# balazs-bamer/cuda-bezier-triangle-raytracer

Hardware: AMD Instinct MI355X
Metric: Mrays/sec (primary+refracted) at 1/2/4/8 MI355X; % of HBM-read roofline (higher is better)
Workload: dtype f32; 1 GPU; cfg4: two stacked cfg2 lenses at x=10 and x=13, 4096x4096 rays; image=4096x4096, primaries_per_gpu=16777216, patches=6144, parallelism=64x64 image tiles round-robin over 1 rank(s), strong scaling, pipeline=fused, frames_in_flight=3, scan=BVH-culled (bit-identical to brute force), numerics=parity: bit-identical to the CPU oracle

## Files before the change

cuda-bezier-triangle-raytracer_amd/bzr_amd/__init__.py:

```python
from __future__ import annotations

import ctypes
import os
from contextlib import contextmanager
from pathlib import Path

import numpy as np

PKG_DIR = Path(__file__).resolve().parent.parent
LIB_PATH = Path(os.environ.get("BZR_LIBRARY", PKG_DIR / "lib" / "libbzr.so"))

OK = 0
HOST_PTRS, DEVICE_PTRS = 0, 1
MODE_PARITY, MODE_FAST = 0, 2
ACCEL_NONE = 4
PIPELINE_STAGED = 8
PIPELINE_FUSED = 16
RAYS_AOS = 32
WHAT_FOLLOW0, WHAT_FOLLOW1, WHAT_FOLLOW2, WHAT_NONE, WHAT_INTERSECT = 0, 1, 2, 3, 4
LIMIT_THIS, LIMIT_NONE = 0, 1
RR_NONE, RR_INSIDE, RR_OUTSIDE = 0, 1, 2
ENVELOPE_ELLIPSOID, ENVELOPE_TESTLENS = 0, 1
PATCH_WORDS = 66
KERNELS = ("k_traverse", "bucket", "k_newton", "k_follow", "k_finish", "k_overflow", "k_intersect_scan",
           "k_refract_scan", "k_chain_scan", "k_patch", "k_newton_lane", "k_trace")
COUNTERS = ("segments", "pairs", "follows", "overflow_rays", "lane_chunks", "node_visits", "leaf_fetches",
            "gate_tests", "newton_rounds", "rounds_odd", "runs_odd", "short_passes")
HIT_FIELDS = 13

_P = ctypes.c_void_p
_U32 = ctypes.c_uint32
_I32 = ctypes.c_int32
_F = ctypes.c_float

_SIGS = {
    "bzr_abi_version": [],
    "bzr_last_error": [],
    "bzr_device_count": [ctypes.POINTER(_I32)],
    "bzr_ctx_create": [_I32, ctypes.POINTER(_P)],
    "bzr_ctx_destroy": [_P],
    "bzr_ctx_set_stream": [_P, _P],
    "bzr_ctx_use_own_stream": [_P],
    "bzr_ctx_get_stream": [_P, ctypes.POINTER(_P)],
    "bzr_sync": [_P],
    "bzr_ctx_timing": [_P, _I32],
    "bzr_ctx_timing_report": [_P, _P, _P],
    "bzr_ctx_counters": [_P, _I32],
    "bzr_ctx_counters_report": [_P, _P],
    "bzr_mesh_create": [_P, _P, _U32, _U32, ctypes.POINTER(_P)],
    "bzr_mesh_destroy": [_P],
    "bzr_mesh_size": [_P, ctypes.POINTER(_U32)],
    "bzr_intersect": [_P, _P, _P, _U32, _P, _U32],
    "bzr_intersect_records": [_P, _P, _P, _U32, _P, _P, _U32],
    "bzr_patch_intersect": [_P, _P, _P, _P, _P, _U32, _P, _U32],
    "bzr_refract": [_P, _P, _F, _P, _P, _U32, _U32, _P, _P, _U32],
    "bzr_trace_chain": [_P, _P, _P, _U32, _P, _U32, _P, _P, _P, _U32],
    "bzr_trace_chain_power": [_P, _P, _P, _U32, _P, _P, _U32, _P, _P, _P, _P, _U32],
    "bzr_trace_chain_spectral": [_P, _P, _P, _U32, _U32, _P, _P, _P, _U32, _P, _P, _P, _P, _U32],
    "bzr_trace_chain_tir": [_P, _P, _P, _U32, _U32, _P, _P, _P, _U32, _U32, _P, _P, _P, _P, _P, _U32],
    "bzr_trace_chain_opl": [_P, _P, _P, _U32, _U32, _P, _P, _P, _P, _U32, _U32, _P, _P, _P, _P, _P, _P, _P, _U32],
    "bzr_trace_chain_media": [_P, _P, _P, _P, _U32, _U32, _P, _P, _P, _P, _U32, _U32, _P, _P, _P, _P, _P, _P, _P, _U32],
    "bzr_dispersion_index": [_I32, _P, _U32, _P, _U32, _P],
    "bzr_trace_tiled": [_P, _U32, _P, _P, _U32, _P, _U32, _U32, _P, _P, _P, _U32],
    "bzr_tiled_create": [_P, _U32, _U32, _U32, _U32, _I32, ctypes.POINTER(_P)],
    "bzr_tiled_destroy": [_P],
    "bzr_tiled_info": [_P, _P, _P, _P],
    "bzr_tiled_set_rays": [_P, _P, _U32],
    "bzr_tiled_share_rays": [_P, _U32, ctypes.POINTER(_P)],
    "bzr_tiled_trace": [_P, _P, _P, _U32, _P, _P, _P, _U32],
    "bzr_tiled_stream": [_P, ctypes.POINTER(_P)],
    "bzr_tiled_sync": [_P],
    "bzr_tiled_set_layout": [_P, _I32, _U32],
    "bzr_tiled_calibrate": [_P, _P, _P, _U32, _U32, ctypes.POINTER(_U32)],
    "bzr_mesh_interpolate": [_P, _P, _I32, _P, _U32],
    "bzr_emit": [_P, _P, ctypes.c_uint64, _U32, _P, _P, _U32],
    "bzr_illuminate": [_P, _P, _P, _U32, _P, ctypes.c_uint64, _P, _P, _P, _U32],
    "bzr_illuminate_power": [_P, _P, _P, _U32, _P, ctypes.c_uint64, _P, _P, _P, _P, _P, _P, _U32],
    "bzr_illuminate_spectral": [_P, _P, _P, _U32, _U32, _P, ctypes.c_uint64, _P, _P, _P, _P, _P, _P, _U32],
    "bzr_illuminate_tir": [_P, _P, _P, _U32, _U32, _P, ctypes.c_uint64, _P, _P, _U32, _P, _P, _P, _P, _P, _P, _P, _P,
                           _U32],
    "bzr_mesh_bounding_sphere": [_P, _P],
    "bzr_trimesh_create": [ctypes.POINTER(_P)],
    "bzr_trimesh_destroy": [_P],
    "bzr_trimesh_copy": [_P, ctypes.POINTER(_P)],
    "bzr_trimesh_size": [_P, ctypes.POINTER(_U32)],
    "bzr_trimesh_get": [_P, _P],
    "bzr_trimesh_set": [_P, _P, _U32],
    "bzr_trimesh_make_solid_of_revolution": [_P, _I32, _I32, _I32, _F, _F, _F],
    "bzr_trimesh_make_ellipsoid": [_P, _I32, _I32, _F, _F, _F],
    "bzr_trimesh_read_stl": [_P, ctypes.c_char_p],
    "bzr_trimesh_write_stl": [_P, ctypes.c_char_p],
    "bzr_trimesh_transform": [_P, _P, _P],
    "bzr_trimesh_split": [_P, _I32],
    "bzr_trimesh_split_maxside": [_P, _F],
    "bzr_trimesh_standardize_vertices": [_P],
    "bzr_trimesh_standardize_normals": [_P],
    "bzr_trimesh_neighbours": [_P, _P, _P],
    "bzr_bezier_build": [_P, _P],
    "bzr_bezier_split_thick": [_P, _P],
    "bzr_bezier_interpolate": [_P, _I32, _P],
    "bzr_pack_frame": [_P, _I32, _P, _P, _P, _U32, _U32, _U32, _P],
    "bzr_debug_unit": [_P, _P, _U32, _P],
    "bzr_debug_div_heights": [_P, _P, _U32, _P],
    "bzr_debug_bundle_setup": [_P, _P, _P, _U32, _P],
    "bzr_debug_fast_unit": [_P, _P, _U32, _P],
    "bzr_debug_wave_clock": [_P, _P, _U32],
    "bzr_debug_wave_clock_rate": [_P, _P, _U32],
    "bzr_debug_chunk_plan": [ctypes.c_uint64, ctypes.c_uint64, ctypes.POINTER(_U32), ctypes.POINTER(_U32)],
    "bzr_debug_chunk_cap": [_P, _U32, ctypes.POINTER(_U32)],
    "bzr_debug_fresnel": [_P, _P, _U32, _P],
}
_ADDED = ("bzr_trace_chain_power", "bzr_illuminate_power", "bzr_trace_chain_spectral", "bzr_illuminate_spectral",
          "bzr_dispersion_index", "bzr_trace_chain_tir", "bzr_illuminate_tir", "bzr_trace_chain_opl",
          "bzr_trace_chain_media")
_RET = {"bzr_last_error": ctypes.c_char_p, "bzr_abi_version": _I32}

_lib = None


class BzrError(RuntimeError):
    pass


def lib():
    global _lib
    if _lib is None:
        if os.environ.get("BZR_NO_TORCH_PRELOAD") != "1":
            try:
                import torch
            except ImportError:
                pass
        if not LIB_PATH.exists():
            raise BzrError(f"{LIB_PATH} is missing: build it with `python -c 'import __graft_entry__ as g; g.build()'`")
        handle = ctypes.CDLL(str(LIB_PATH))
        for name, args in _SIGS.items():
            if (os.environ.get("BZR_LIBRARY") and (name.startswith("bzr_debug_") or name in _ADDED)
                    and not hasattr(handle, name)):
                continue
            fn = getattr(handle, name)
            fn.argtypes = args
            fn.restype = _RET.get(name, _I32)
        _lib = handle
    return _lib


def exported_symbols():
    return list(_SIGS)


def _check(status: int):
    if status != OK:
        msg = lib().bzr_last_error().decode(errors="replace")
        raise BzrError(f"libbzr status {status}: {msg}")


def device_count() -> int:
    c = _I32(0)
    _check(lib().bzr_device_count(ctypes.byref(c)))
    return c.value


def _is_tensor(x) -> bool:
    return hasattr(x, "data_ptr") and hasattr(x, "is_cuda")


class _Buf:

    def __init__(self, x, dtype, writable=False):
        if x is None:
            self.ptr, self.device, self.keep = None, None, None
            return
        if _is_tensor(x):
            if not x.is_contiguous():
                raise BzrError("tensor arguments must be contiguous")
            want = {np.float32: "torch.float32", np.uint32: "torch.uint32", np.int32: "torch.int32",
                    np.uint64: "torch.uint64", np.uint8: "torch.uint8"}
            same_bits = {np.uint32: "torch.int32", np.uint64: "torch.int64"}
            if str(x.dtype) not in (want[dtype], same_bits.get(dtype, want[dtype])):
                raise BzrError(f"tensor dtype {x.dtype} where {want[dtype]} is expected")
            self.ptr, self.device, self.keep = x.data_ptr(), bool(x.is_cuda), x
        else:
            a = np.asarray(x)
            if a.dtype != dtype or not a.flags["C_CONTIGUOUS"]:
                if writable:
                    raise BzrError(f"output array must be C-contiguous {np.dtype(dtype).name}")
                a = np.ascontiguousarray(a, dtype=dtype)
            self.ptr, self.device, self.keep = a.ctypes.data, False, a
# ... 756 lines not shown
```

cuda-bezier-triangle-raytracer_amd/csrc/device/patch_math.hpp:

```cpp
#pragma once
#include <hip/hip_runtime.h>
#include <cfloat>
#include <cstdint>

namespace bzr_dev {

struct f3 {
  float x, y, z;
};
__device__ __forceinline__ f3 mk(float x, float y, float z) { return f3{x, y, z}; }
namespace rec {
constexpr int kUnder = 0;
constexpr int kDivider = 4;
constexpr int kNeigh = 16;
constexpr int kCp = 19;
constexpr int kMinv = 49;
constexpr int kHin = 58;
constexpr int kHout = 59;
constexpr int kDirA = 60;
constexpr int kDirB = 63;
constexpr int kWords = 66;
}

struct Patch {
// ... 73 lines not shown
#ifndef BZR_NEWTON_UNROLL
#define BZR_NEWTON_UNROLL 1
#endif
constexpr uint32_t kFollow2 = 2u, kNone = 3u, kIntersect = 4u;

namespace exact {
__device__ __forceinline__ float div_rn(float a, float b) { return a / b; }
__device__ __forceinline__ float sqrt_rn(float a) { return __builtin_sqrtf(a); }

__device__ __forceinline__ float sqrt_unscaled(float z) {
  const float s = __builtin_amdgcn_sqrtf(z);
  const float lo = __uint_as_float(__float_as_uint(s) - 1u), hi = __uint_as_float(__float_as_uint(s) + 1u);
  const float rlo = __builtin_fmaf(-lo, s, z), rhi = __builtin_fmaf(-hi, s, z);
  const float t = rlo <= 0.0f ? lo : s;
  return rhi > 0.0f ? hi : t;
}
__device__ __forceinline__ float div_unscaled(float a, float b, float y) {
  float q = a * y;
  float r = __builtin_fmaf(-b, q, a);
  q = __builtin_fmaf(r, y, q);
  r = __builtin_fmaf(-b, q, a);
  return __builtin_fmaf(r, y, q);
}
__device__ __forceinline__ bool sqrt_above_hundredth(float z) { return z > __uint_as_float(0x38d1b718u); }
__device__ __forceinline__ f3 unit_or_self(f3 a, float z) {
  const float s = sqrt_unscaled(z);
  const float y0 = __builtin_amdgcn_rcpf(s);
  const float y = __builtin_fmaf(__builtin_fmaf(-s, y0, 1.0f), y0, y0);
  f3 r = mk(div_unscaled(a.x, s, y), div_unscaled(a.y, s, y), div_unscaled(a.z, s, y));
  const float m = fminf(fminf(fabsf(a.x), fabsf(a.y)), fabsf(a.z));
  if (!(m >= 0x1p-100f && z >= 0x1p-96f && z <= 0x1p40f)) {
    r = a;
    if (z > 0.0f) {
      const float sr = sqrt_rn(z);
      r = mk(div_rn(a.x, sr), div_rn(a.y, sr), div_rn(a.z, sr));
    }
  }
  return r;
}
#ifndef BZR_DIV_HEIGHTS
#define BZR_DIV_HEIGHTS 1
#endif
__device__ __forceinline__ bool height_in_range(float h) {
  const uint32_t e = (__float_as_uint(h) >> 23) & 0xFFu;
  return e - (127u - 40u) <= 80u;
}
__device__ __forceinline__ void div_heights(float hin, float hout, float ic, float &din, float &dout) {
#if BZR_DIV_HEIGHTS
  const bool ok = height_in_range(hin) && height_in_range(hout) && fabsf(ic) >= 0x1p-20f && fabsf(ic) <= 0x1p20f;
  if (__all(ok)) {
    const float y0 = __builtin_amdgcn_rcpf(ic);
    const float y = __builtin_fmaf(__builtin_fmaf(-ic, y0, 1.0f), y0, y0);
    din = div_unscaled(hin, ic, y);
    dout = div_unscaled(hout, ic, y);
    return;
  }
#endif
  din = div_rn(hin, ic);
  dout = div_rn(hout, ic);
}
#include "patch_math_body.inc"
}

namespace fast {
#pragma clang fp contract(fast)
__device__ __forceinline__ float div_rn(float a, float b) { return a * __builtin_amdgcn_rcpf(b); }
__device__ __forceinline__ float sqrt_rn(float a) { return __builtin_amdgcn_sqrtf(a); }
__device__ __forceinline__ bool sqrt_above_hundredth(float z) { return sqrt_rn(z) > 0.01f; }
__device__ __forceinline__ f3 unit_or_self(f3 a, float z) {
  if (!(z > 0.0f)) return a;
  float r = __builtin_amdgcn_rsqf(z);
  return mk(a.x * r, a.y * r, a.z * r);
}
__device__ __forceinline__ void div_heights(float hin, float hout, float ic, float &din, float &dout) {
  din = div_rn(hin, ic);
  dout = div_rn(hout, ic);
}
#include "patch_math_body.inc"
#pragma clang fp contract(off)
}

using namespace exact;

template <bool kGated = false, bool kFast = false, typename P, typename Need = NormalAlways>
__device__ __forceinline__ Hit patch_intersect(const P &p, f3 s, f3 d, bool limitNone, Need need = Need()) {
  Hit h;
  h.t = 0.0f;
  h.point = mk(0.0f, 0.0f, 0.0f);
  h.cs = 0.0f;
  h.bary = h.point;
  h.normal = h.point;
  h.what = kNone;
  f3 ip;
  float ic, it;
  bool valid = plane_ray(p.n(), p.c(), s, d, ip, ic, it);
  (void)valid;
  if (!kGated) {
    if (!(valid && fabsf(it) > -p.hin() && fabsf(it) > p.hout())) return h;
    f3 b0 = matvec(p, ip);
    if (!(limitNone || (b0.x >= 0.0f && b0.x <= 1.0f && b0.y >= 0.0f && b0.y <= 1.0f && b0.z >= 0.0f && b0.z <= 1.0f)))
      return h;
  }
  if constexpr (kFast) return fast::newton_tail(p, s, d, ic, it, need);
  else return newton_tail(p, s, d, ic, it, need);
}

}
```

cuda-bezier-triangle-raytracer_amd/csrc/device/trace.hip:

```cpp
#include <hip/hip_runtime.h>
#include <hipcub/hipcub.hpp>

#include <algorithm>
#include <climits>
#include <cmath>
#include <cstdlib>

#include <cstdio>
#include <cstring>
#include <new>
#include <type_traits>
#include <string>
#include <vector>

#include "../host/bvh.hpp"
#include "../host/staging.hpp"
#include "bzr.h"
#include "ctx.hpp"
#include "patch_math.hpp"
#include "emitter.hpp"

using namespace bzr_dev;

namespace {
thread_local std::string t_error;
bzr_status set_error(bzr_status s, const std::string &msg) {
  t_error = msg;
  return s;
}
#define BZR_HIP(call)                                                                                     \
  do {                                                                                                    \
    hipError_t e_ = (call);                                                                               \
    if (e_ != hipSuccess) return set_error(BZR_ERR_HIP, std::string(#call ": ") + hipGetErrorString(e_)); \
  } while (0)
}

extern "C" const char *bzr_last_error(void) { return t_error.c_str(); }
extern "C" int32_t bzr_abi_version(void) { return BZR_ABI_VERSION; }
extern "C" void bzr_internal_set_error(const char *msg) { t_error = msg ? msg : ""; }

struct bzr_mesh {
  int device;
  uint32_t n;
  float4 *planar;
  float *full;
  bzr_host::Bvh4Node *nodes;
  float4 *leaf;
  bzr_host::Bvh4Node *nodes_near;
  float4 *leaf_near;
  bzr_host::Bvh4ObbNode *obb;
  bzr_host::Bvh4ObbNode *obb_near;
  float4 *kids;
  float4 *kids_near;
  float4 *wide;
  float4 *wide_near;
  float4 *swide;
  float4 *swide_near;
  uint32_t split;
  float4 *always;
  uint32_t n_always;
  uint32_t nnodes;
  float s_max;
  float s_near;
  float sphere[4];
};

namespace {

constexpr int kBlock = 256;
constexpr int kWaves = kBlock / 64;
constexpr uint32_t kMaxLenses = 8;
constexpr uint32_t kMaxCand = 40;
constexpr uint32_t kOverflow = 0x8000u;
#ifndef BZR_STACK
#define BZR_STACK 64
#endif
constexpr int kStack = BZR_STACK;
constexpr uint32_t kCounterReplicas = 64;

typedef uint32_t u32x16 __attribute__((ext_vector_type(16)));
typedef __attribute__((address_space(4))) const u32x16 cu32x16;

constexpr uint32_t kXcds = 8;
__device__ __forceinline__ uint32_t xcd_contiguous(uint32_t b, uint32_t nblocks) {
  const uint32_t q = nblocks / kXcds, r = nblocks % kXcds, x = b % kXcds;
  return x * q + (x < r ? x : r) + b / kXcds;
}
#ifndef BZR_TRAV_ABLOCK
#define BZR_TRAV_ABLOCK 1
#endif
static_assert(BZR_TRAV_ABLOCK == 0 || BZR_TRAV_ABLOCK == 1, "BZR_TRAV_ABLOCK: 0 or 1");
#ifndef BZR_ABLOCK_BLOCK
#define BZR_ABLOCK_BLOCK 256
#endif
constexpr uint32_t kAblockMin = 64, kAblockMax = 1024, kAblockBlock = BZR_ABLOCK_BLOCK;
constexpr int kTravBlock = 64;
constexpr float kBundleSpread = 0.5f;
constexpr uint32_t kWideSlots = 16u;
#ifndef BZR_TRACE_WIDE
#define BZR_TRACE_WIDE 1
#endif
constexpr uint32_t kOverflowBlocks = 2048u;
// ... 1417 lines not shown
template <>
struct TraceKeep<kModeMedia> : TraceKeep<kModeOpl> {};
template <int kMode>
constexpr bool kSplitWalk = BZR_TRACE_BUNDLE && BZR_TRACE_WIDE && (kMode == kModeRefract || kMode == kModeStage);
template <bool kOn>
struct TraceSeen {};
template <>
struct TraceSeen<true> {
  alignas(16) uint32_t seen[bzr_host::kSplitSlotCap / 32];
};
template <int kMode>
struct TraceLds : TraceKeep<kMode>, TraceSeen<kSplitWalk<kMode>> {
  uint32_t stack[TraceWords<kMode>::kStackCap];
  float hit[TraceWords<kMode>::kHit][64];
  unsigned long long emask[kEntries];
  float bundle[kBundleWords];
  uint32_t eid[kEntries];
#if BZR_TRACE_SHORT == 1
  uint32_t ekey[kEntries];
#endif
#if BZR_TRACE_BUNDLE
  uint32_t pend[64];
#endif
  float park[TraceWords<kMode>::kPark ? TraceWords<kMode>::kPark : 1][64];
};

__device__ __forceinline__ unsigned long long uniform_u64(unsigned long long v) {
  const uint32_t hi = __builtin_amdgcn_readfirstlane((uint32_t)(v >> 32)), lo = __builtin_amdgcn_readfirstlane((uint32_t)v);
  return ((unsigned long long)hi << 32) | lo;
}

template <int kMode>
__device__ __forceinline__ void consider(const Hit &h, uint32_t scan, uint32_t src, unsigned long long &best,
                                         TraceLds<kMode> &L, uint32_t lane) {
  if (h.what == kIntersect && h.t < FLT_MAX) {
    const unsigned long long k = ((unsigned long long)t_order(h.t) << 32) | scan;
    if (k < best) {
      best = k;
      if constexpr (kMode == kModeHits) {
        L.hit[0][lane] = h.t;
        L.hit[1][lane] = h.point.x;
        L.hit[2][lane] = h.point.y;
        L.hit[3][lane] = h.point.z;
        L.hit[4][lane] = h.cs;
        L.hit[5][lane] = h.bary.x;
        L.hit[6][lane] = h.bary.y;
        L.hit[7][lane] = h.bary.z;
        L.hit[8][lane] = h.normal.x;
        L.hit[9][lane] = h.normal.y;
        L.hit[10][lane] = h.normal.z;
        L.hit[11][lane] = __uint_as_float(src);
      } else {
        L.hit[0][lane] = h.point.x;
        L.hit[1][lane] = h.point.y;
        L.hit[2][lane] = h.point.z;
        L.hit[3][lane] = h.cs;
        L.hit[4][lane] = h.normal.x;
        L.hit[5][lane] = h.normal.y;
        L.hit[6][lane] = h.normal.z;
      }
    }
  }
}

struct PassVote {
  unsigned long long best;
  uint32_t scan;
  bool spec;
  bool *skipped;
  __device__ __forceinline__ bool operator()(float t) const {
#if BZR_TRACE_SHORT
    const bool may = spec || (t < FLT_MAX && (((unsigned long long)t_order(t) << 32) | scan) < best);
    const bool any = __any(may);
    *skipped = !any;
    return any;
#else
    (void)t;
    return true;
#endif
  }
};

__device__ __forceinline__ uint32_t entry_key(float gt, unsigned long long pm) {
  return t_order(__int_as_float(__builtin_amdgcn_readlane(__float_as_int(gt), (int)__builtin_ctzll(pm))));
}

template <int kMode>
__device__ __forceinline__ Hit winner(TraceLds<kMode> &L, uint32_t lane, uint32_t &patch) {
  Hit h = no_hit();
  h.what = kIntersect;
  if constexpr (kMode == kModeHits) {
    h.t = L.hit[0][lane];
    h.point = mk(L.hit[1][lane], L.hit[2][lane], L.hit[3][lane]);
    h.cs = L.hit[4][lane];
    h.bary = mk(L.hit[5][lane], L.hit[6][lane], L.hit[7][lane]);
    h.normal = mk(L.hit[8][lane], L.hit[9][lane], L.hit[10][lane]);
    patch = __float_as_uint(L.hit[11][lane]);
  } else {
    h.point = mk(L.hit[0][lane], L.hit[1][lane], L.hit[2][lane]);
    h.cs = L.hit[3][lane];
    h.normal = mk(L.hit[4][lane], L.hit[5][lane], L.hit[6][lane]);
    patch = 0xFFFFFFFFu;
  }
  return h;
}

template <int kMode>
__device__ __forceinline__ void park(const Hit &h, TraceLds<kMode> &L, uint32_t lane) {
  if constexpr (TraceWords<kMode>::kPark > 0) {
    L.park[0][lane] = h.what == kIntersect ? h.t : __uint_as_float(0x7FC00000u);
    L.park[1][lane] = h.point.x;
    L.park[2][lane] = h.point.y;
    L.park[3][lane] = h.point.z;
    L.park[4][lane] = h.cs;
    L.park[5][lane] = h.normal.x;
    L.park[6][lane] = h.normal.y;
    L.park[7][lane] = h.normal.z;
    if constexpr (TraceWords<kMode>::kPark >= 11) {
      L.park[8][lane] = h.bary.x;
      L.park[9][lane] = h.bary.y;
      L.park[10][lane] = h.bary.z;
    }
  }
}
template <int kMode>
__device__ __forceinline__ Hit parked(TraceLds<kMode> &L, uint32_t lane) {
  Hit h = no_hit();
  if constexpr (TraceWords<kMode>::kPark > 0) {
    h.t = L.park[0][lane];
    h.point = mk(L.park[1][lane], L.park[2][lane], L.park[3][lane]);
    h.cs = L.park[4][lane];
    h.normal = mk(L.park[5][lane], L.park[6][lane], L.park[7][lane]);
    if constexpr (TraceWords<kMode>::kPark >= 11) h.bary = mk(L.park[8][lane], L.park[9][lane], L.park[10][lane]);
    h.what = kIntersect;
  }
  return h;
}

template <int kMode, bool kFast, bool kCount>
__device__ __forceinline__ void trace_segment(const MeshView &m, f3 s, f3 d, bool act, unsigned long long &best,
                                              TraceLds<kMode> &L, uint32_t lane, TraceCtr &ctr) {
  constexpr bool kPark = TraceWords<kMode>::kPark > 0;
  constexpr uint32_t kNo = 0xFFFFFFFFu;
  constexpr int kCap = TraceWords<kMode>::kStackCap;
  constexpr bool kOrder = BZR_TRACE_SHORT == 1;
  best = ~0ull;
  const float amax = fmaxf(fmaxf(fabsf(s.x), fabsf(s.y)), fabsf(s.z));
  bool ovf = false;
  if (act && !(amax <= m.s_max)) {
    ovf = true;
    act = false;
  }
  const bool near_tier = !__any(act && !(amax <= m.s_near));
  const bzr_host::Bvh4Node *nodes = near_tier ? m.nodes_near : m.nodes;
  const bzr_host::Bvh4ObbNode *obb = near_tier ? m.obb_near : m.obb;
  const float4 *leaf = near_tier ? m.leaf_near : m.leaf;
  const f3 inv = mk(safe_inv(d.x), safe_inv(d.y), safe_inv(d.z));
  const f3 sinv = mk(s.x * inv.x, s.y * inv.y, s.z * inv.z);
  int sp = 0;
  uint32_t next = (m.n > 0 && __any(act)) ? 0u : kNo;
  unsigned long long next_hm = 0ull;
  uint32_t scan = kNo;
  uint32_t join = kNo, join_src = 0;
  uint32_t parked_nb = kNo;
  uint32_t ab = (m.n_always && __any(act)) ? 0u : (m.n_always + 63u) / 64u;
  unsigned long long am = 0ull;
  bool bwalk = false;
#if BZR_TRACE_BUNDLE
  uint32_t npend = 0, pi = 0;
  const float4 *kids = near_tier ? m.kids_near : m.kids;
  bool narrow = false;
  if (next != kNo) {
    narrow = bundle_setup_swap(act, s, d, L.bundle, lane) <= kBundleSpread;
    if constexpr (kSplitWalk<kMode>) {
      static_assert(sizeof(L.seen) == 64 * sizeof(uint4), "one uint4 per lane clears the slot set");
      if (narrow && m.split > 1u) reinterpret_cast<uint4 *>(L.seen)[lane] = make_uint4(0u, 0u, 0u, 0u);
    }
    if (lane == 0u) L.stack[0] = 0u;
    sp = 1;
    next = kNo;
    bwalk = true;
  }
#endif
  for (;;) {
    uint32_t ne = 0;
    __builtin_amdgcn_s_setprio(3);
#if BZR_TRACE_BUNDLE
    while (bwalk && ne < kEntries) {
      if (pi < npend) {
        const uint32_t slot = __builtin_amdgcn_readfirstlane(L.pend[pi]);
        ++pi;
        const u32x16 r = *((const cu32x16 *)(uintptr_t)leaf + slot);
        float gt;
        const bool pass = act & planar_gate(leaf_q(r, 0), leaf_q(r, 1), leaf_q(r, 2), leaf_q(r, 3), s, d, gt);
        if (kCount) {
          ++ctr.leaves;
          ctr.gate_tests += popc64(__ballot(act));
        }
        const unsigned long long pm = __ballot(pass);
        if (pm) {
          const uint32_t key = kOrder ? entry_key(gt, pm) : 0u;
          (void)key;
          if (lane == 0u) {
            L.eid[ne] = r[15];
            L.emask[ne] = pm;
#if BZR_TRACE_SHORT == 1
            L.ekey[ne] = key;
#endif
          }
          ++ne;
        }
        continue;
      }
      if (sp == 0) break;
      pi = npend = 0;
      const uint32_t top = __builtin_amdgcn_readfirstlane(L.stack[sp - 1]);
      if (!narrow || (top & bzr_host::kObbFlag)) {
        --sp;
        if (kCount) ++ctr.nodes;
        bool hit[4];
        uint32_t ch[4];
        const f3 linv = mk(safe_inv(d.x), safe_inv(d.y), safe_inv(d.z));
        node_children(nodes, obb, top, act, s, d, mk(s.x * linv.x, s.y * linv.y, s.z * linv.z), linv, hit, ch);
#pragma unroll
        for (int c = 0; c < 4; ++c) {
          const unsigned long long hm = __ballot(hit[c]);
          if (hm == 0ull) continue;
          if (ch[c] & bzr_host::kLeafFlag) {
            if (lane == 0u) L.pend[npend] = ch[c] & ~bzr_host::kLeafFlag;
            ++npend;
          } else if (sp < kCap) {
            if (lane == 0u) L.stack[sp] = ch[c];
            ++sp;
          } else if (lane_bit(hm, lane)) {
            ovf = true;
          }
        }
        continue;
      }
      bool full;
      uint32_t k;
#if BZR_TRACE_WIDE
      if constexpr (kSplitWalk<kMode>)
        npend = bundle_batch<kCap, 16>(near_tier ? m.swide_near : m.swide, L.stack, sp, L.pend, L.bundle, lane, full, k,
                                       0u, m.split > 1u ? L.seen : nullptr);
      else
        npend = bundle_batch<kCap, 16>(near_tier ? m.wide_near : m.wide, L.stack, sp, L.pend, L.bundle, lane, full, k);
#else
      npend = bundle_batch<kCap>(kids, L.stack, sp, L.pend, L.bundle, lane, full, k);
#endif
      if (full) ovf |= act;
      if (kCount) ctr.nodes += k;
    }
#else
    while ((next != kNo || sp > 0) && ne + 4u <= kEntries) {
      const uint32_t node = next != kNo ? next : __builtin_amdgcn_readfirstlane(L.stack[--sp]);
      next = kNo;
      if (kCount) ++ctr.nodes;
      bool hit[4];
      uint32_t ch[4];
      node_children(nodes, obb, node, act, s, d, sinv, inv, hit, ch);
#pragma unroll
      for (int c = 0; c < 4; ++c) {
        const unsigned long long hm = __ballot(hit[c]);
        if (hm == 0ull) continue;
        if (ch[c] & bzr_host::kLeafFlag) {
          const u32x16 r = *((const cu32x16 *)(uintptr_t)leaf + (ch[c] & ~bzr_host::kLeafFlag));
          const float4 g0 = make_float4(__uint_as_float(r[0]), __uint_as_float(r[1]), __uint_as_float(r[2]), __uint_as_float(r[3]));
          const float4 g1 = make_float4(__uint_as_float(r[4]), __uint_as_float(r[5]), __uint_as_float(r[6]), __uint_as_float(r[7]));
          const float4 g2 = make_float4(__uint_as_float(r[8]), __uint_as_float(r[9]), __uint_as_float(r[10]), __uint_as_float(r[11]));
          const float4 g3 = make_float4(__uint_as_float(r[12]), __uint_as_float(r[13]), __uint_as_float(r[14]), 0.0f);
          float gt;
          const bool pass = hit[c] & planar_gate(g0, g1, g2, g3, s, d, gt);
          if (kCount) {
            ++ctr.leaves;
            ctr.gate_tests += popc64(hm);
          }
          const unsigned long long pm = __ballot(pass);
          if (pm) {
            const uint32_t key = kOrder ? entry_key(gt, pm) : 0u;
            (void)key;
            if (lane == 0u) {
              L.eid[ne] = r[15];
              L.emask[ne] = pm;
#if BZR_TRACE_SHORT == 1
              L.ekey[ne] = key;
#endif
            }
            ++ne;
          }
        } else {
          if (next != kNo) {
            if (sp < kCap) L.stack[sp++] = next;
            else if (lane_bit(next_hm, lane)) ovf = true;
          }
          next = ch[c];
          next_hm = hm;
        }
      }
    }
#endif
    while (next == kNo && sp == 0 && ne < kEntries) {
      if (am == 0ull) {
        if (ab * 64u >= m.n_always) break;
        if (ab == 0u && !BZR_TRACE_BUNDLE) bundle_to_lds(act, s, d, L.bundle, lane);
        am = __ballot(always_bundle_keep(m.always, ab * 64u + lane, m.n_always, L.bundle));
        ++ab;
        continue;
      }
      const uint32_t k = (ab - 1u) * 64u + __builtin_ctzll(am);
      am &= am - 1ull;
      uint32_t b;
      float gt;
      const bool pass = always_gate(m.always, k, act, s, d, b, gt);
      if (kCount) {
        ++ctr.leaves;
        ctr.gate_tests += popc64(__ballot(act));
      }
      const unsigned long long pm = __ballot(pass);
      if (pm) {
        const uint32_t key = kOrder ? entry_key(gt, pm) : 0u;
        (void)key;
        if (lane == 0u) {
          L.eid[ne] = b;
          L.emask[ne] = pm;
#if BZR_TRACE_SHORT == 1
          L.ekey[ne] = key;
#endif
        }
        ++ne;
      }
    }
    if (ne == 0u) {
#define BZR_SEG_END break;
      if (scan == kNo) {
        if (!__any(ovf)) BZR_SEG_END
        scan = 0;
        if (kCount) ctr.ovf += popc64(__ballot(ovf));
      }
      bool pass = false;
      for (; scan < m.n; ++scan) {
        const float4 *g = m.planar + 4u * scan;
        pass = ovf && planar_gate(g[0], g[1], g[2], g[3], s, d);
        if (__any(pass)) break;
      }
      if (scan >= m.n) BZR_SEG_END
#undef BZR_SEG_END
      const unsigned long long pm = __ballot(pass);
      if (lane == 0u) {
        L.eid[0] = scan;
        L.emask[0] = pm;
      }
      ne = 1;
      ++scan;
    }
    __builtin_amdgcn_s_setprio(0);
    if (kOrder && ne >= 2u) {
      const uint32_t slot = lane & (kEntries - 1u);
#if BZR_TRACE_SHORT == 1
      const uint32_t ekey = L.ekey[slot];
#else
      const uint32_t ekey = 0u;
#endif
      uint32_t rank = 0;
      for (uint32_t j = 0; j < ne; ++j) {
        const uint32_t kj = (uint32_t)__builtin_amdgcn_readlane((int)ekey, (int)j);
        rank += (kj < ekey || (kj == ekey && j < lane)) ? 1u : 0u;
      }
      const uint32_t id = L.eid[slot];
      const unsigned long long em = L.emask[slot];
      __builtin_amdgcn_wave_barrier();
      if (lane < ne) {
        L.eid[rank] = id;
        L.emask[rank] = em;
      }
      __builtin_amdgcn_wave_barrier();
    }
    for (uint32_t e = 0; e < ne; ++e) {
      const uint32_t b = __builtin_amdgcn_readfirstlane(L.eid[e]);
      const auto hp = uniform_patch(m.full, b);
      const bool run0 = lane_bit(uniform_u64(L.emask[e]), lane);
      const bool joined = join == b;
      const uint32_t sidx = joined ? join_src : b;
      if (joined) join = kNo;
      bool spec = false;
      if (kPark && e + 1u < ne) {
        unsigned long long sm = 0ull;
#pragma unroll
        for (uint32_t side = 0; side < 3u; ++side) {
          const uint32_t nb = __float_as_uint(hp.r[rec::kNeigh + side]);
          const unsigned long long later = __ballot(lane > e && lane < ne && L.eid[lane & (kEntries - 1u)] == nb);
          if (later) sm |= uniform_u64(L.emask[__builtin_ctzll(later)]);
        }
        spec = lane_bit(sm, lane) && !run0 && !joined && parked_nb == kNo;
      }
      if (kCount) {
        ++ctr.rounds;
        ctr.pairs += popc64(__ballot(run0));
        ctr.follows += popc64(__ballot(joined));
      }
      uint32_t what = kNone;
      bool skipped = false;
      if (run0 || joined || spec) {
        const Hit h = patch_intersect<false, kFast>(hp, s, d, joined || spec, PassVote{best, sidx, spec, &skipped});
        if (spec) {
          park(h, L, lane);
          parked_nb = b;
        } else {
          consider(h, sidx, b, best, L, lane);
          if (!joined) what = h.what;
        }
      }
      if (kCount && __any(skipped)) ++ctr.shorts;
      for (uint32_t side = 0; side < 3u; ++side) {
        bool fl = run0 && what == side;
        if (!__any(fl)) continue;
        const uint32_t nb = __float_as_uint(hp.r[rec::kNeigh + side]);
        if (kPark) {
          const bool use = fl && parked_nb == nb;
          if (use) {
            consider(parked(L, lane), b, nb, best, L, lane);
            fl = false;
          }
          if (kCount) ctr.follows += popc64(__ballot(use));
          if (!__any(fl)) continue;
        }
        const unsigned long long later = __ballot(lane > e && lane < ne && L.eid[lane & (kEntries - 1u)] == nb);
        if (later) {
          const unsigned long long fm = uniform_u64(L.emask[__builtin_ctzll(later)]);
          if (fl && join == kNo && !lane_bit(fm, lane)) {
            join = nb;
            join_src = b;
            fl = false;
          }
        }
        if (!__any(fl)) continue;
        if (kCount) {
          ++ctr.rounds;
          ctr.follows += popc64(__ballot(fl));
        }
        const auto pa = uniform_patch(m.full, nb);
        skipped = false;
        if (fl) {
          const Hit h = patch_intersect<false, kFast>(pa, s, d, true, PassVote{best, b, false, &skipped});
          consider(h, b, nb, best, L, lane);
        }
        if (kCount && __any(skipped)) ++ctr.shorts;
      }
    }
  }
}

struct TraceJob {
  const float *rays;
  float *hits;
  float *out_rays;
  uint32_t *status;
  uint32_t *segments;
  const uint32_t *expected;
  const uint32_t *alive_in;
  uint32_t expected_all;
  uint32_t n;
  uint32_t ld;
  unsigned long long *wave_clock;
  uint32_t wave_real;
  const uint32_t *order;
  uint32_t *cost;
  float *weight;
  const float *weight_in;
  const uint8_t *channel;
  const float *ri_table;
  uint32_t nchan;
  uint32_t lossless;
  uint32_t *bounces;
  uint32_t max_bounces;
  float *opl;
  const float *opl_in;
  float *glass;
  const float *gap_table;
};

constexpr int kTraceWpe = 6;
#define BZR_TRACE_ATTR __attribute__((amdgpu_waves_per_eu(kTraceWpe)))
constexpr int kTraceBlock = 64, kTraceWaves = kTraceBlock / 64;
#ifndef BZR_TRACE_SCHED
#define BZR_TRACE_SCHED 1
#endif
#ifndef BZR_TRACE_SCHED_REFRESH
#define BZR_TRACE_SCHED_REFRESH 16
#endif
#ifndef BZR_TRACE_SCHED_OCT
#define BZR_TRACE_SCHED_OCT 4
#endif
constexpr uint32_t kSchedBins = 128, kSchedMinTiles = 2048, kSchedThreads = 256;
__device__ __forceinline__ uint32_t sched_bin(unsigned long long cycles) {
  const uint32_t c = static_cast<uint32_t>(cycles > 0xFFFFFFFFull ? 0xFFFFFFFFull : cycles) | 4u;
  const uint32_t lg = 31u - __clz(c);
  constexpr uint32_t kSub = BZR_TRACE_SCHED_OCT == 4 ? 2u : (BZR_TRACE_SCHED_OCT == 2 ? 1u : 0u);
  const uint32_t key = 4u * lg + (((c >> (lg - 2u)) & 3u) >> (2u - kSub) << (2u - kSub));
  return kSchedBins - 1u - key;
}
__global__ __launch_bounds__(kSchedThreads) void k_sched_count(const uint32_t *__restrict__ bin, uint32_t tiles,
                                                               uint32_t *__restrict__ hist) {
  __shared__ uint32_t h[kSchedBins];
  for (uint32_t k = threadIdx.x; k < kSchedBins; k += kSchedThreads) h[k] = 0u;
  __syncthreads();
  const uint32_t t = blockIdx.x * kSchedThreads + threadIdx.x;
  if (t < tiles) atomicAdd(&h[bin[t] & (kSchedBins - 1u)], 1u);
  __syncthreads();
  for (uint32_t k = threadIdx.x; k < kSchedBins; k += kSchedThreads)
// ... 1418 lines not shown
extern "C" bzr_status bzr_trace_chain_spectral(bzr_ctx *ctx, const bzr_mesh *const *lenses, const float *ri_table,
                                               uint32_t nlens, uint32_t nchan, const float *rays, const uint8_t *channel,
                                               const float *weight_in, uint32_t n, float *out_rays, float *out_weight,
                                               uint32_t *out_status, uint32_t *out_segments, uint32_t flags) {
  return trace_chain<kModeSpectral>(ctx, lenses, ri_table, nlens, rays, weight_in, n, out_rays, out_weight, out_status,
                                    out_segments, flags, channel, nchan);
}

extern "C" bzr_status bzr_trace_chain_tir(bzr_ctx *ctx, const bzr_mesh *const *lenses, const float *ri_table,
                                          uint32_t nlens, uint32_t nchan, const float *rays, const uint8_t *channel,
                                          const float *weight_in, uint32_t n, uint32_t max_bounces, float *out_rays,
                                          float *out_weight, uint32_t *out_status, uint32_t *out_segments,
                                          uint32_t *out_bounces, uint32_t flags) {
  return trace_chain<kModeTir>(ctx, lenses, ri_table, nlens, rays, weight_in, n, out_rays, out_weight, out_status,
                               out_segments, flags, channel, nchan, max_bounces, out_bounces);
}

extern "C" bzr_status bzr_trace_chain_opl(bzr_ctx *ctx, const bzr_mesh *const *lenses, const float *ri_table,
                                          uint32_t nlens, uint32_t nchan, const float *rays, const uint8_t *channel,
                                          const float *weight_in, const float *opl_in, uint32_t n, uint32_t max_bounces,
                                          float *out_rays, float *out_weight, uint32_t *out_status,
                                          uint32_t *out_segments, uint32_t *out_bounces, float *out_opl, float *out_glass,
                                          uint32_t flags) {
  if (!out_opl) return set_error(BZR_ERR_INVALID_ARGUMENT, "null out_opl");
  if (max_bounces > BZR_MAX_BOUNCES) return set_error(BZR_ERR_INVALID_ARGUMENT, "max_bounces must be 0..8");
  return trace_chain<kModeOpl>(ctx, lenses, ri_table, nlens, rays, weight_in, n, out_rays, out_weight, out_status,
                               out_segments, flags, channel, nchan, max_bounces, out_bounces, opl_in, out_opl, out_glass);
}

extern "C" bzr_status bzr_trace_chain_media(bzr_ctx *ctx, const bzr_mesh *const *lenses, const float *ri_table,
                                            const float *gap_table, uint32_t nlens, uint32_t nchan, const float *rays,
                                            const uint8_t *channel, const float *weight_in, const float *opl_in,
                                            uint32_t n, uint32_t max_bounces, float *out_rays, float *out_weight,
                                            uint32_t *out_status, uint32_t *out_segments, uint32_t *out_bounces,
                                            float *out_opl, float *out_glass, uint32_t flags) {
  if (!out_opl) return set_error(BZR_ERR_INVALID_ARGUMENT, "null out_opl");
  if (max_bounces > BZR_MAX_BOUNCES) return set_error(BZR_ERR_INVALID_ARGUMENT, "max_bounces must be 0..8");
  return trace_chain<kModeMedia>(ctx, lenses, ri_table, nlens, rays, weight_in, n, out_rays, out_weight, out_status,
                                 out_segments, flags, channel, nchan, max_bounces, out_bounces, opl_in, out_opl, out_glass,
                                 gap_table);
}

namespace {
__global__ __launch_bounds__(kBlock) void k_debug_unit(const float *__restrict__ a, uint32_t n,
                                                       float *__restrict__ out) {
  const uint32_t i = blockIdx.x * kBlock + threadIdx.x;
  if (i >= n) return;
  const f3 v = mk(a[i], a[(size_t)n + i], a[(size_t)2 * n + i]);
  const f3 u = normalized(v);
  const float z = dot(v, v);
  f3 w = v;
  if (z > 0.0f) {
    const float s = sqrt_rn(z);
    w = mk(div_rn(v.x, s), div_rn(v.y, s), div_rn(v.z, s));
  }
  const float r[6] = {u.x, u.y, u.z, w.x, w.y, w.z};
#pragma unroll
  for (int k = 0; k < 6; ++k) out[(size_t)k * n + i] = r[k];
}
__global__ __launch_bounds__(kBlock) void k_debug_div_heights(const float *__restrict__ a, uint32_t n,
                                                              float *__restrict__ out) {
  const uint32_t i = blockIdx.x * kBlock + threadIdx.x;
  if (i >= n) return;
  const float hin = a[i], hout = a[(size_t)n + i], ic = a[(size_t)2 * n + i];
  float din, dout;
  div_heights(hin, hout, ic, din, dout);
  out[i] = din;
  out[(size_t)n + i] = dout;
  out[(size_t)2 * n + i] = div_rn(hin, ic);
  out[(size_t)3 * n + i] = div_rn(hout, ic);
}
__global__ __launch_bounds__(64) void k_debug_bundle_setup(const float *__restrict__ rays,
                                                           const uint8_t *__restrict__ active, uint32_t n,
                                                           float *__restrict__ out) {
  __shared__ float bl[kBundleWords];
  const uint32_t lane = threadIdx.x, i = blockIdx.x * 64u + lane;
  const f3 s = mk(rays[i], rays[(size_t)n + i], rays[(size_t)2 * n + i]);
  const f3 d = mk(rays[(size_t)3 * n + i], rays[(size_t)4 * n + i], rays[(size_t)5 * n + i]);
  const float spread = bundle_setup_swap(active[i] != 0, s, d, bl, lane);
  float *o = out + (size_t)blockIdx.x * (kBundleWords + 1u);
  if (lane < kBundleWords) o[lane] = bl[lane];
  if (lane == kBundleWords) o[lane] = spread;
}
__global__ __launch_bounds__(kBlock) void k_debug_fast_unit(const float *__restrict__ a, uint32_t n,
                                                            float *__restrict__ out) {
  const uint32_t i = blockIdx.x * kBlock + threadIdx.x;
  if (i >= n) return;
  const f3 v = mk(a[i], a[(size_t)n + i], a[(size_t)2 * n + i]);
  const f3 u = fast::normalized(v);
  const float r[5] = {fast::div_rn(v.x, v.y), fast::sqrt_rn(fabsf(v.x)), u.x, u.y, u.z};
#pragma unroll
  for (int k = 0; k < 5; ++k) out[(size_t)k * n + i] = r[k];
}
}

extern "C" bzr_status bzr_debug_fast_unit(void *ctxp, const float *a, uint32_t n, float *out) {
  bzr_ctx *ctx = static_cast<bzr_ctx *>(ctxp);
  if (!ctx) return set_error(BZR_ERR_INVALID_ARGUMENT, "null context");
  if (n == 0) return BZR_OK;
  if (!a || !out) return set_error(BZR_ERR_INVALID_ARGUMENT, "null buffer");
  DeviceGuard g(ctx->device);
  hipLaunchKernelGGL(k_debug_fast_unit, dim3((n + kBlock - 1) / kBlock), dim3(kBlock), 0, ctx->stream, a, n, out);
  BZR_HIP(hipGetLastError());
  return BZR_OK;
}

extern "C" bzr_status bzr_debug_div_heights(void *ctxp, const float *a, uint32_t n, float *out) {
  bzr_ctx *ctx = static_cast<bzr_ctx *>(ctxp);
  if (!ctx) return set_error(BZR_ERR_INVALID_ARGUMENT, "null context");
  if (n == 0) return BZR_OK;
  if (!a || !out) return set_error(BZR_ERR_INVALID_ARGUMENT, "null buffer");
  DeviceGuard g(ctx->device);
  hipLaunchKernelGGL(k_debug_div_heights, dim3((n + kBlock - 1) / kBlock), dim3(kBlock), 0, ctx->stream, a, n, out);
  BZR_HIP(hipGetLastError());
  return BZR_OK;
}

extern "C" bzr_status bzr_debug_bundle_setup(void *ctxp, const float *rays, const uint8_t *active, uint32_t n,
                                             float *out) {
  bzr_ctx *ctx = static_cast<bzr_ctx *>(ctxp);
  if (!ctx) return set_error(BZR_ERR_INVALID_ARGUMENT, "null context");
  if (n == 0) return BZR_OK;
  if (!rays || !active || !out) return set_error(BZR_ERR_INVALID_ARGUMENT, "null buffer");
  if (n % 64u) return set_error(BZR_ERR_INVALID_ARGUMENT, "n must be whole waves of 64 rays");
  DeviceGuard g(ctx->device);
  hipLaunchKernelGGL(k_debug_bundle_setup, dim3(n / 64u), dim3(64), 0, ctx->stream, rays, active, n, out);
  BZR_HIP(hipGetLastError());
  return BZR_OK;
}

extern "C" bzr_status bzr_debug_chunk_plan(uint64_t free_bytes, uint64_t n, uint32_t *cap, uint32_t *chunk) {
  if (!cap || !chunk) return set_error(BZR_ERR_INVALID_ARGUMENT, "null argument");
  *cap = chunk_cap_of(free_bytes);
  *chunk = chunk_len(n, *cap);
  return BZR_OK;
}

extern "C" bzr_status bzr_debug_chunk_cap(void *ctxp, uint32_t rays, uint32_t *effective) {
  bzr_ctx *ctx = static_cast<bzr_ctx *>(ctxp);
  if (!ctx) return set_error(BZR_ERR_INVALID_ARGUMENT, "null context");
  DeviceGuard g(ctx->device);
  ctx->chunk_limit = rays ? std::max(rays / 64u * 64u, 64u) : 0u;
  if (effective) *effective = chunk_cap(ctx);
  return BZR_OK;
}

extern "C" bzr_status bzr_debug_wave_clock(void *ctxp, unsigned long long *clock, uint32_t waves) {
  bzr_ctx *ctx = static_cast<bzr_ctx *>(ctxp);
  if (!ctx) return set_error(BZR_ERR_INVALID_ARGUMENT, "null context");
  ctx->wave_clock = clock;
  ctx->wave_clock_cap = clock ? waves : 0u;
  ctx->wave_clock_real = false;
  return BZR_OK;
}

extern "C" bzr_status bzr_debug_wave_clock_rate(void *ctxp, unsigned long long *clock, uint32_t waves) {
  bzr_ctx *ctx = static_cast<bzr_ctx *>(ctxp);
  if (!ctx) return set_error(BZR_ERR_INVALID_ARGUMENT, "null context");
  ctx->wave_clock = clock;
  ctx->wave_clock_cap = clock ? waves : 0u;
  ctx->wave_clock_real = clock != nullptr;
  return BZR_OK;
}

extern "C" bzr_status bzr_debug_unit(void *ctxp, const float *a, uint32_t n, float *out) {
  bzr_ctx *ctx = static_cast<bzr_ctx *>(ctxp);
  if (!ctx) return set_error(BZR_ERR_INVALID_ARGUMENT, "null context");
  if (n == 0) return BZR_OK;
  if (!a || !out) return set_error(BZR_ERR_INVALID_ARGUMENT, "null buffer");
  DeviceGuard g(ctx->device);
  hipLaunchKernelGGL(k_debug_unit, dim3((n + kBlock - 1) / kBlock), dim3(kBlock), 0, ctx->stream, a, n, out);
  BZR_HIP(hipGetLastError());
  return BZR_OK;
}

extern "C" uint32_t bzr_internal_unit_subtriangles(int32_t divisor, float *out);

namespace {
__global__ __launch_bounds__(kBlock) void k_tessellate(const float *__restrict__ full, uint32_t nb,
                                                       const float *__restrict__ bary, uint64_t total,
                                                       float *__restrict__ out) {
  const uint64_t t = (uint64_t)blockIdx.x * kBlock + threadIdx.x;
  if (t >= total) return;
  const uint32_t k = static_cast<uint32_t>(t / nb), b = static_cast<uint32_t>(t % nb);
  const PatchView<const float *> p{full + (size_t)rec::kWords * b};
  const float *bk = bary + (size_t)9 * k;
#pragma unroll
  for (int v = 0; v < 3; ++v) {
    const f3 q = interpolate(p, mk(bk[3 * v], bk[3 * v + 1], bk[3 * v + 2]));
    out[(size_t)9 * t + 3 * v] = q.x;
    out[(size_t)9 * t + 3 * v + 1] = q.y;
    out[(size_t)9 * t + 3 * v + 2] = q.z;
  }
}
}

extern "C" bzr_status bzr_mesh_interpolate(bzr_ctx *ctx, const bzr_mesh *mesh, int32_t divisor, float *out_xyz,
                                           uint32_t flags) {
  if (bzr_status s = check_flags(flags)) return s;
  if (bzr_status s = check_ctx_mesh(ctx, mesh)) return s;
  if (divisor < 1 || divisor > 4096) return set_error(BZR_ERR_INVALID_ARGUMENT, "divisor must be 1..4096");
  const uint32_t K = static_cast<uint32_t>(divisor) * static_cast<uint32_t>(divisor);
  const uint64_t total = (uint64_t)K * mesh->n;
  if (total == 0) return BZR_OK;
  if (!out_xyz) return set_error(BZR_ERR_INVALID_ARGUMENT, "null buffer");
  DeviceGuard g(ctx->device);
  std::vector<float> bary((size_t)K * 9);
  if (bzr_internal_unit_subtriangles(divisor, bary.data()) != K)
    return set_error(BZR_ERR_INVALID_ARGUMENT, "sub-triangle count mismatch");
// ... 515 lines not shown
```

include/bzr_debug.h:

```cpp
#ifndef BZR_DEBUG_H
#define BZR_DEBUG_H
#include <stdint.h>
#ifdef __cplusplus
extern "C" {
#endif
int32_t bzr_debug_gate_boxes(const void *patches, uint32_t n, uint32_t stride, float *boxes, float *s_max);
int32_t bzr_debug_gate_boxes_tier(const void *patches, uint32_t n, uint32_t stride, int32_t tier, float *boxes,
                                  float *s_max);
int32_t bzr_debug_always_list(const void *patches, uint32_t n, uint32_t stride, int32_t tier, uint32_t *out,
                              uint32_t *count);
int32_t bzr_debug_always_wedges(const void *patches, uint32_t n, uint32_t stride, int32_t tier, float *out);
int32_t bzr_debug_gate_obbs(const void *patches, uint32_t n, uint32_t stride, int32_t tier, float *out);
int32_t bzr_debug_bounding_sphere(const void *patches, uint32_t n, uint32_t stride, float out[4]);
int32_t bzr_debug_traverse(const void *patches, uint32_t n, uint32_t stride, const float *rays, uint32_t nr,
                           uint8_t *hits, uint64_t stats[4]);
int32_t bzr_debug_traverse_bundle(const void *patches, uint32_t n, uint32_t stride, const float *rays, uint32_t nr,
                                  float max_spread, uint64_t stats[12]);
int32_t bzr_debug_traverse_bundle_split(const void *patches, uint32_t n, uint32_t stride, const float *rays, uint32_t nr,
                                        float max_spread, int32_t split, uint64_t stats[16], uint32_t *slots);
int32_t bzr_debug_split_boxes(const void *patches, uint32_t n, uint32_t stride, int32_t tier, int32_t split,
                              uint32_t *patch, float *boxes, uint32_t *count, uint32_t *order, float *patch_box);
int32_t bzr_debug_region_points(const void *patches, uint32_t n, uint32_t stride, int32_t tier, uint32_t *patch,
                                double *pts, uint32_t *count);
int32_t bzr_debug_nodes4(const void *patches, uint32_t n, uint32_t stride, int32_t tier, int32_t split, void *out,
                         uint32_t *count);
int32_t bzr_debug_unit(void *ctx, const float *a, uint32_t n, float *out);
int32_t bzr_debug_div_heights(void *ctx, const float *a, uint32_t n, float *out);
int32_t bzr_debug_bundle_setup(void *ctx, const float *rays, const uint8_t *active, uint32_t n, float *out);
int32_t bzr_debug_fast_unit(void *ctx, const float *a, uint32_t n, float *out);
int32_t bzr_debug_chunk_plan(uint64_t free_bytes, uint64_t n, uint32_t *cap, uint32_t *chunk);
int32_t bzr_debug_chunk_cap(void *ctx, uint32_t rays, uint32_t *effective);
int32_t bzr_debug_wave_clock(void *ctx, unsigned long long *clock, uint32_t waves);
int32_t bzr_debug_wave_clock_rate(void *ctx, unsigned long long *clock, uint32_t waves);
int32_t bzr_debug_newton_short(const void *patches, uint32_t n, uint32_t stride, const uint32_t *patch,
                               const float *rays, const uint8_t *limit, uint32_t m, float *full, float *skipped);
int32_t bzr_debug_fresnel(const float *eta, const float *cs, uint32_t n, float *t_out);
#ifdef __cplusplus
}
#endif
#endif
```

Before: 12510 Mrays/s.

## Order batch entries by insertion into nibble-packed order word; skip redundant barycentric gate

```diff
diff --git a/cuda-bezier-triangle-raytracer_amd/bzr_amd/__init__.py b/cuda-bezier-triangle-raytracer_amd/bzr_amd/__init__.py
--- a/cuda-bezier-triangle-raytracer_amd/bzr_amd/__init__.py
+++ b/cuda-bezier-triangle-raytracer_amd/bzr_amd/__init__.py
@@ -103,6 +103,7 @@
     "bzr_debug_unit": [_P, _P, _U32, _P],
     "bzr_debug_div_heights": [_P, _P, _U32, _P],
     "bzr_debug_bundle_setup": [_P, _P, _P, _U32, _P],
+    "bzr_debug_pass_order": [_P, _P, _P, _U32, _P],
     "bzr_debug_fast_unit": [_P, _P, _U32, _P],
     "bzr_debug_wave_clock": [_P, _P, _U32],
     "bzr_debug_wave_clock_rate": [_P, _P, _U32],
diff --git a/cuda-bezier-triangle-raytracer_amd/csrc/device/pass_order.hpp b/cuda-bezier-triangle-raytracer_amd/csrc/device/pass_order.hpp
--- /dev/null
+++ b/cuda-bezier-triangle-raytracer_amd/csrc/device/pass_order.hpp
@@ -0,0 +1,20 @@
+#pragma once
+#include <cstdint>
+
+#if defined(__HIPCC__)
+#define BZR_ORDER_FN __host__ __device__ __forceinline__
+#else
+#define BZR_ORDER_FN inline
+#endif
+
+namespace bzr_dev {
+
+constexpr uint32_t kOrderEntries = 16;
+
+BZR_ORDER_FN uint64_t order_insert(uint64_t order, uint32_t e, uint32_t front) {
+  const uint64_t below = (uint64_t(1) << (4u * front)) - 1u;
+  return (order & below) | (uint64_t(e) << (4u * front)) | ((order & ~below) << 4);
+}
+BZR_ORDER_FN uint32_t order_at(uint64_t order, uint32_t p) { return uint32_t(order >> (4u * p)) & 15u; }
+
+}
diff --git a/cuda-bezier-triangle-raytracer_amd/csrc/device/patch_math.hpp b/cuda-bezier-triangle-raytracer_amd/csrc/device/patch_math.hpp
--- a/cuda-bezier-triangle-raytracer_amd/csrc/device/patch_math.hpp
+++ b/cuda-bezier-triangle-raytracer_amd/csrc/device/patch_math.hpp
@@ -179,7 +179,8 @@
 
 using namespace exact;
 
-template <bool kGated = false, bool kFast = false, typename P, typename Need = NormalAlways>
+constexpr int kGateFull = 0, kGateDone = 1, kGatePlane = 2;
+template <int kGated = kGateFull, bool kFast = false, typename P, typename Need = NormalAlways>
 __device__ __forceinline__ Hit patch_intersect(const P &p, f3 s, f3 d, bool limitNone, Need need = Need()) {
   Hit h;
   h.t = 0.0f;
@@ -192,14 +193,24 @@
   float ic, it;
   bool valid = plane_ray(p.n(), p.c(), s, d, ip, ic, it);
   (void)valid;
-  if (!kGated) {
+  if (kGated != kGateDone) {
     if (!(valid && fabsf(it) > -p.hin() && fabsf(it) > p.hout())) return h;
-    f3 b0 = matvec(p, ip);
-    if (!(limitNone || (b0.x >= 0.0f && b0.x <= 1.0f && b0.y >= 0.0f && b0.y <= 1.0f && b0.z >= 0.0f && b0.z <= 1.0f)))
-      return h;
+    if (kGated == kGateFull) {
+      f3 b0 = matvec(p, ip);
+      if (!(limitNone || (b0.x >= 0.0f && b0.x <= 1.0f && b0.y >= 0.0f && b0.y <= 1.0f && b0.z >= 0.0f && b0.z <= 1.0f)))
+        return h;
+    }
   }
   if constexpr (kFast) return fast::newton_tail(p, s, d, ic, it, need);
   else return newton_tail(p, s, d, ic, it, need);
 }
-
-}
+template <typename P>
+__device__ __forceinline__ bool patch_gate(const P &p, f3 s, f3 d) {
+  f3 ip;
+  float ic, it;
+  if (!(plane_ray(p.n(), p.c(), s, d, ip, ic, it) && fabsf(it) > -p.hin() && fabsf(it) > p.hout())) return false;
+  const f3 b0 = matvec(p, ip);
+  return b0.x >= 0.0f && b0.x <= 1.0f && b0.y >= 0.0f && b0.y <= 1.0f && b0.z >= 0.0f && b0.z <= 1.0f;
+}
+
+}
diff --git a/cuda-bezier-triangle-raytracer_amd/csrc/device/trace.hip b/cuda-bezier-triangle-raytracer_amd/csrc/device/trace.hip
--- a/cuda-bezier-triangle-raytracer_amd/csrc/device/trace.hip
+++ b/cuda-bezier-triangle-raytracer_amd/csrc/device/trace.hip
@@ -18,6 +18,7 @@
 #include "bzr.h"
 #include "ctx.hpp"
 #include "patch_math.hpp"
+#include "pass_order.hpp"
 #include "emitter.hpp"
 
 using namespace bzr_dev;
@@ -1601,7 +1602,26 @@
 };
 
 __device__ __forceinline__ uint32_t entry_key(float gt, unsigned long long pm) {
-  return t_order(__int_as_float(__builtin_amdgcn_readlane(__float_as_int(gt), (int)__builtin_ctzll(pm))));
+  return (uint32_t)__builtin_amdgcn_readlane(__float_as_int(gt), (int)__builtin_ctzll(pm));
+}
+static_assert(kEntries <= kOrderEntries, "a batch's order is one word of nibbles (pass_order.hpp)");
+template <bool kOrder, typename Lds>
+__device__ __forceinline__ void batch_append(Lds &L, uint32_t ne, unsigned long long &order, uint32_t id,
+                                             unsigned long long pm, uint32_t key, uint32_t lane) {
+  uint32_t front = ne;
+  if constexpr (kOrder) {
+    front = 0u;
+    if (ne) {
+      __builtin_amdgcn_wave_barrier();
+      front = popc64(__ballot(L.ekey[lane & (kEntries - 1u)] <= key) & ((1ull << ne) - 1ull));
+    }
+  }
+  order = order_insert(order, ne, front);
+  if (lane == 0u) {
+    L.eid[ne] = id;
+    L.emask[ne] = pm;
+    if constexpr (kOrder) L.ekey[ne] = key;
+  }
 }
 
 template <int kMode>
@@ -1703,6 +1723,7 @@
 #endif
   for (;;) {
     uint32_t ne = 0;
+    unsigned long long order = 0ull;
     __builtin_amdgcn_s_setprio(3);
 #if BZR_TRACE_BUNDLE
     while (bwalk && ne < kEntries) {
@@ -1718,15 +1739,7 @@
         }
         const unsigned long long pm = __ballot(pass);
         if (pm) {
-          const uint32_t key = kOrder ? entry_key(gt, pm) : 0u;
-          (void)key;
-          if (lane == 0u) {
-            L.eid[ne] = r[15];
-            L.emask[ne] = pm;
-#if BZR_TRACE_SHORT == 1
-            L.ekey[ne] = key;
-#endif
-          }
+          batch_append<kOrder>(L, ne, order, r[15], pm, kOrder ? entry_key(gt, pm) : 0u, lane);
           ++ne;
         }
         continue;
@@ -1797,15 +1810,7 @@
           }
           const unsigned long long pm = __ballot(pass);
           if (pm) {
-            const uint32_t key = kOrder ? entry_key(gt, pm) : 0u;
-            (void)key;
-            if (lane == 0u) {
-              L.eid[ne] = r[15];
-              L.emask[ne] = pm;
-#if BZR_TRACE_SHORT == 1
-              L.ekey[ne] = key;
-#endif
-            }
+            batch_append<kOrder>(L, ne, order, r[15], pm, kOrder ? entry_key(gt, pm) : 0u, lane);
             ++ne;
           }
         } else {
@@ -1838,15 +1843,7 @@
       }
       const unsigned long long pm = __ballot(pass);
       if (pm) {
-        const uint32_t key = kOrder ? entry_key(gt, pm) : 0u;
-        (void)key;
-        if (lane == 0u) {
-          L.eid[ne] = b;
-          L.emask[ne] = pm;
-#if BZR_TRACE_SHORT == 1
-          L.ekey[ne] = key;
-#endif
-        }
+        batch_append<kOrder>(L, ne, order, b, pm, kOrder ? entry_key(gt, pm) : 0u, lane);
         ++ne;
       }
     }
@@ -1874,54 +1871,36 @@
       ++scan;
     }
     __builtin_amdgcn_s_setprio(0);
-    if (kOrder && ne >= 2u) {
-      const uint32_t slot = lane & (kEntries - 1u);
-#if BZR_TRACE_SHORT == 1
-      const uint32_t ekey = L.ekey[slot];
-#else
-      const uint32_t ekey = 0u;
-#endif
-      uint32_t rank = 0;
-      for (uint32_t j = 0; j < ne; ++j) {
-        const uint32_t kj = (uint32_t)__builtin_amdgcn_readlane((int)ekey, (int)j);
-        rank += (kj < ekey || (kj == ekey && j < lane)) ? 1u : 0u;
-      }
-      const uint32_t id = L.eid[slot];
-      const unsigned long long em = L.emask[slot];
-      __builtin_amdgcn_wave_barrier();
-      if (lane < ne) {
-        L.eid[rank] = id;
-        L.emask[rank] = em;
-      }
-      __builtin_amdgcn_wave_barrier();
-    }
-    for (uint32_t e = 0; e < ne; ++e) {
-      const uint32_t b = __builtin_amdgcn_readfirstlane(L.eid[e]);
+    for (uint32_t todo = (1u << ne) - 1u; todo; order >>= 4) {
+      const uint32_t ei = order_at(order, 0u);
+      todo ^= 1u << ei;
+      const bool more = todo != 0u;
+      const uint32_t b = __builtin_amdgcn_readfirstlane(L.eid[ei]);
       const auto hp = uniform_patch(m.full, b);
-      const bool run0 = lane_bit(uniform_u64(L.emask[e]), lane);
+      const bool run0 = lane_bit(uniform_u64(L.emask[ei]), lane);
       const bool joined = join == b;
       const uint32_t sidx = joined ? join_src : b;
       if (joined) join = kNo;
       bool spec = false;
-      if (kPark && e + 1u < ne) {
+      if (kPark && more) {
         unsigned long long sm = 0ull;
 #pragma unroll
         for (uint32_t side = 0; side < 3u; ++side) {
           const uint32_t nb = __float_as_uint(hp.r[rec::kNeigh + side]);
-          const unsigned long long later = __ballot(lane > e && lane < ne && L.eid[lane & (kEntries - 1u)] == nb);
+          const unsigned long long later = __ballot(L.eid[lane & (kEntries - 1u)] == nb) & todo;
           if (later) sm |= uniform_u64(L.emask[__builtin_ctzll(later)]);
         }
         spec = lane_bit(sm, lane) && !run0 && !joined && parked_nb == kNo;
       }
       if (kCount) {
         ++ctr.rounds;
-        ctr.pairs += popc64(__ballot(run0));
+        ctr.pairs += popc64(__ballot(run0 && patch_gate(hp, s, d)));
         ctr.follows += popc64(__ballot(joined));
       }
       uint32_t what = kNone;
       bool skipped = false;
       if (run0 || joined || spec) {
-        const Hit h = patch_intersect<false, kFast>(hp, s, d, joined || spec, PassVote{best, sidx, spec, &skipped});
+        const Hit h = patch_intersect<kGatePlane, kFast>(hp, s, d, joined || spec, PassVote{best, sidx, spec, &skipped});
         if (spec) {
           park(h, L, lane);
           parked_nb = b;
@@ -1944,7 +1923,7 @@
           if (kCount) ctr.follows += popc64(__ballot(use));
           if (!__any(fl)) continue;
         }
-        const unsigned long long later = __ballot(lane > e && lane < ne && L.eid[lane & (kEntries - 1u)] == nb);
+        const unsigned long long later = __ballot(L.eid[lane & (kEntries - 1u)] == nb) & todo;
         if (later) {
           const unsigned long long fm = uniform_u64(L.emask[__builtin_ctzll(later)]);
           if (fl && join == kNo && !lane_bit(fm, lane)) {
@@ -3529,6 +3508,30 @@
   if (lane < kBundleWords) o[lane] = bl[lane];
   if (lane == kBundleWords) o[lane] = spread;
 }
+constexpr unsigned long long kDebugBallot = 0x9E3779B97F4A7C15ull;
+struct DebugBatchLds {
+  unsigned long long emask[kEntries];
+  uint32_t eid[kEntries];
+  uint32_t ekey[kEntries];
+};
+__global__ __launch_bounds__(64) void k_debug_pass_order(const uint32_t *__restrict__ keys,
+                                                         const uint32_t *__restrict__ len, uint32_t *__restrict__ out) {
+  __shared__ DebugBatchLds L;
+  const uint32_t lane = threadIdx.x, w = blockIdx.x;
+  const uint32_t n = min(__builtin_amdgcn_readfirstlane(len[w]), kEntries);
+  unsigned long long order = 0ull;
+  for (uint32_t e = 0; e < n; ++e)
+    batch_append<true>(L, e, order, e, kDebugBallot * (e + 1u), __builtin_amdgcn_readfirstlane(keys[kEntries * w + e]),
+                       lane);
+  __builtin_amdgcn_wave_barrier();
+  if (lane < kEntries) {
+    const uint32_t ei = order_at(order, lane);
+    uint32_t *o = out + (size_t)3 * (kEntries * w + lane);
+    o[0] = lane < n ? L.eid[ei] : 0xFFFFFFFFu;
+    o[1] = lane < n ? (uint32_t)L.emask[ei] : 0xFFFFFFFFu;
+    o[2] = lane < n ? (uint32_t)(L.emask[ei] >> 32) : 0xFFFFFFFFu;
+  }
+}
 __global__ __launch_bounds__(kBlock) void k_debug_fast_unit(const float *__restrict__ a, uint32_t n,
                                                             float *__restrict__ out) {
   const uint32_t i = blockIdx.x * kBlock + threadIdx.x;
@@ -3572,6 +3575,18 @@
   if (n % 64u) return set_error(BZR_ERR_INVALID_ARGUMENT, "n must be whole waves of 64 rays");
   DeviceGuard g(ctx->device);
   hipLaunchKernelGGL(k_debug_bundle_setup, dim3(n / 64u), dim3(64), 0, ctx->stream, rays, active, n, out);
+  BZR_HIP(hipGetLastError());
+  return BZR_OK;
+}
+
+extern "C" bzr_status bzr_debug_pass_order(void *ctxp, const uint32_t *keys, const uint32_t *len, uint32_t n,
+                                           uint32_t *out) {
+  bzr_ctx *ctx = static_cast<bzr_ctx *>(ctxp);
+  if (!ctx) return set_error(BZR_ERR_INVALID_ARGUMENT, "null context");
+  if (n == 0) return BZR_OK;
+  if (!keys || !len || !out) return set_error(BZR_ERR_INVALID_ARGUMENT, "null buffer");
+  DeviceGuard g(ctx->device);
+  hipLaunchKernelGGL(k_debug_pass_order, dim3(n), dim3(64), 0, ctx->stream, keys, len, out);
   BZR_HIP(hipGetLastError());
   return BZR_OK;
 }
diff --git a/include/bzr_debug.h b/include/bzr_debug.h
--- a/include/bzr_debug.h
+++ b/include/bzr_debug.h
@@ -27,6 +27,7 @@
 int32_t bzr_debug_unit(void *ctx, const float *a, uint32_t n, float *out);
 int32_t bzr_debug_div_heights(void *ctx, const float *a, uint32_t n, float *out);
 int32_t bzr_debug_bundle_setup(void *ctx, const float *rays, const uint8_t *active, uint32_t n, float *out);
+int32_t bzr_debug_pass_order(void *ctx, const uint32_t *keys, const uint32_t *len, uint32_t n, uint32_t *out);
 int32_t bzr_debug_fast_unit(void *ctx, const float *a, uint32_t n, float *out);
 int32_t bzr_debug_chunk_plan(uint64_t free_bytes, uint64_t n, uint32_t *cap, uint32_t *chunk);
 int32_t bzr_debug_chunk_cap(void *ctx, uint32_t rays, uint32_t *effective);
```

Result: faster. 12820 Mrays/s (median of 6 runs) (+2.5%).
